# BoloniniD/CSWin-UNet

Hardware: AMD Instinct MI355X
Metric: training images/sec (224x224, cswin_tiny) (higher is better)
Workload: dtype f32; 1 GPU; cswin_tiny_224_lite, synthetic 224x224 9-class, bs=24/GPU, fp32 matmul, fwd + 0.4CE+0.6Dice + bwd + SGD(momentum) step, drop_path 0.2; global_batch=24, img_size=224, parallelism=dp1, hip_graph=True

## Files before the change

### cswin_unet_amd/_lib.py

```python
import ctypes
import os
from ctypes import c_char_p, c_double, c_float, c_int, c_long, c_size_t, c_void_p

import torch

_HERE = os.path.dirname(os.path.abspath(__file__))
LIB_PATH = os.path.join(_HERE, "libcswin_hip.so")

P, I, F, SZ, L, D = c_void_p, c_int, c_float, c_size_t, c_long, c_double

ABI_VERSION = 4

SIGNATURES = {
    "cswin_last_error": (c_char_p, []),
    "cswin_abi_version": (I, []),
    "cswin_device_ok": (I, []),
    "cswin_attn_fwd": (I, [P, P, P, P, P, P, I, I, I, I, P, P, I, F, F, ctypes.c_ulonglong, P, I, P]),
    "cswin_attn_bwd_workspace": (SZ, [I, I, I, I, P, P, I]),
    "cswin_attn_bwd": (I, [P, P, P, P, P, P, P, P, P, P, SZ, I, I, I, I, P, P, I, F, P, F, ctypes.c_ulonglong, P, I, P]),
    "cswin_img2windows": (I, [P, P, I, I, I, I, I, I, P]),
    "cswin_windows2img": (I, [P, P, I, I, I, I, I, I, P]),
    "cswin_layernorm_fwd": (I, [P, P, P, P, P, P, I, I, F, I, P]),
    "cswin_layernorm_bwd_workspace": (SZ, [I, I]),
    "cswin_layernorm_bwd": (I, [P, P, P, P, P, P, P, P, P, P, SZ, I, I, P, P, P]),
    "cswin_linear_fwd": (I, [P, P, I, P, P, P, P, P, P, I, I, I, I, I, I, P]),
    "cswin_linear_bwd_data": (I, [P, P, P, P, I, P, P, I, P, I, I, I, I, I, P]),
    "cswin_linear_bwd_weight_workspace": (SZ, [I, I, I]),
    "cswin_linear_bwd_weight": (I, [P, P, P, I, P, I, P, P, P, SZ, I, I, I, P, I, P]),
    "cswin_linear_bwd_weight_batch": (I, [P, I, P, P, I, P]),
    "cswin_linear_bwd_tail": (I, [P, P, P, I, I, I, P, I, P, P, I, P]),
    "cswin_rows_sum_multi": (I, [P, I, P]),
    "cswin_conv_tok_fwd": (I, [P, P, P, P, I, I, I, I, I, I, I, I, I, P]),
    "cswin_conv_tok_bwd_data": (I, [P, P, P, I, I, I, I, I, I, I, I, I, P]),
    "cswin_conv_tok_bwd_weight_workspace": (SZ, [I, I, I, I, I, I, I, I]),
    "cswin_conv_tok_bwd_weight": (I, [P, P, P, P, P, SZ, I, I, I, I, I, I, I, I, I, P, I, P]),
    "cswin_conv_weight_permute": (I, [P, P, P, I, I, I, I, P]),
    "cswin_conv_weight_unpermute": (I, [P, P, I, I, I, I, P]),
    "cswin_conv_weight_flipT": (I, [P, P, I, I, I, P]),
    "cswin_conv_weight_images": (I, [P, I, P]),
    "cswin_conv_tok_bwd_weight_cpad": (I, [P, P, P, P, P, SZ, I, I, I, I, I, I, I, I, I, P, I, P]),
    "cswin_nchw_to_tokens": (I, [P, P, I, I, I, I, I, P]),
    "cswin_tokens_to_nchw": (I, [P, P, I, I, I, I, I, P]),
    "cswin_carafe_fwd": (I, [P, P, P, P, P, I, I, I, I, I, P]),
    "cswin_carafe_bwd_workspace": (SZ, [I, I, I, I, I]),
    "cswin_carafe_bwd": (I, [P, P, P, P, P, P, P, SZ, I, I, I, I, I, P, P]),
# ... 183 lines not shown
```

### cswin_unet_amd/csrc/gemm.hip

```cpp
#include <stdlib.h>

#include <type_traits>
#include "common.h"
#include "gemm_epilogue.h"

int cswin_gemm16(int mode, int epi_mode, const void* A, const void* B, const void* epilogue, int M, int NO, int R, void* stream);
int cswin_wgrad16_batch(const cswin_wgrad_desc* d, int n, const int* splits, const int* rows_per_split, const cswin_reduce_job* pending,
                        int npending, void* stream, long long* stamps);

namespace {

constexpr int BKMAX = 64;

typedef __bf16 bf16x8 __attribute__((ext_vector_type(8)));
typedef __bf16 bf16x4 __attribute__((ext_vector_type(4)));

#define CSWIN_CHECK_PRECISION(p, who) CSWIN_REQUIRE((p) == 0 || (p) == 1, CSWIN_ERR_UNSUPPORTED, who ": precision %d (0 = fp32, 1 = bf16 operands)", (p))

struct PlainSrc {
    const float* p; long ld; int rows, cols;
    const float* row_scale; int rows_per_sample;
    int bf16;
    static constexpr bool fast_div = false;
    struct Row { const float* base; float s; };
// ... 2 lines not shown
    __device__ Row row(int i) const {
        Row r;
        r.base = (i < rows) ? p + (long)i * ld : nullptr;
        r.s = (row_scale && i < rows) ? row_scale[i / rows_per_sample] : 1.0f;
        return r;
    }
    __device__ const float* ptr(const Row& r, int j) const { return (r.base && j < cols) ? r.base + j : nullptr; }
};

template <class S> __device__ __forceinline__ bool src_is_bf16(const S&) { return false; }
__device__ __forceinline__ bool src_is_bf16(const PlainSrc& s) { return s.bf16 != 0; }
template <class S> __device__ __forceinline__ u32x2 src_load4_bf16(const S&, const float*) { return u32x2{0u, 0u}; }
__device__ __forceinline__ u32x2 src_load4_bf16(const PlainSrc& s, const float* p) {
    return *reinterpret_cast<const u32x2*>(reinterpret_cast<const __bf16*>(s.p) + (p - s.p));
}

struct ConcatSrc {
    const float* p0; const float* p1; long ld0, ld1; int rows, cols, c0;
    static constexpr bool fast_div = false;
    struct Row { const float* b0; const float* b1; float s; };
    typedef int Col;
    __device__ Col col(int j) const { return j; }
    __device__ Row row(int i) const {
        Row r;
        r.b0 = (i < rows) ? p0 + (long)i * ld0 : nullptr;
        r.b1 = (i < rows) ? p1 + (long)i * ld1 : nullptr;
        r.s = 1.0f;
        return r;
    }
    __device__ const float* ptr(const Row& r, int j) const {
// ... 132 lines not shown
        return r;
    }
    __device__ Col col(int j) const { return j; }
    __device__ const float* ptr(const Row& r, int j) const { return (r.base && j < cols) ? r.base + j : nullptr; }
};

template <int BM, int BN, int BK, int KW, bool A_RC, bool B_RC>
constexpr int gemm_lds_floats() {
    constexpr int NW = (BM >= 64 ? 2 : 1) * (BN >= 64 ? 2 : 1);
    constexpr int LDR = BK + 4;
    constexpr int A_ELEMS = A_RC ? BM * LDR : BK * (BM + 4);
    constexpr int B_ELEMS = B_RC ? BN * LDR : BK * (BN + 4);
    return (A_ELEMS + B_ELEMS) > NW * EP_WAVE_FLOATS ? (A_ELEMS + B_ELEMS) : NW * EP_WAVE_FLOATS;
}

template <int BM, int BN, int BK, int KW, bool A_RC, bool B_RC, int VEC, int EPI, bool SCALE_A, int PREC, class ASrc, class BSrc>
__device__ __forceinline__ void gemm_body(float* lds, const ASrc& A, const BSrc& B, const Epilogue& epi, int M, int N, int R,
                                          int r_per_split, int tiles_m, int tiles_n, int bid, int nblk, int stamp_row) {
    constexpr int WGM = BM >= 64 ? 2 : 1, WGN = BN >= 64 ? 2 : 1, NW = WGM * WGN;
    constexpr int WM = BM / WGM, WN = BN / WGN;
    constexpr int FM = WM / 32, FN = WN / 32;
    constexpr int LDR = BK + 4;
    constexpr int LDA = A_RC ? LDR : BM + 4;
    constexpr int LDB = B_RC ? LDR : BN + 4;
    constexpr int A_ELEMS = A_RC ? BM * LDR : BK * (BM + 4);
    constexpr int B_ELEMS = B_RC ? BN * LDR : BK * (BN + 4);
    constexpr int LDS_FLOATS = gemm_lds_floats<BM, BN, BK, KW, A_RC, B_RC>();
    static_assert(LDS_FLOATS >= A_ELEMS + B_ELEMS && LDS_FLOATS >= NW * EP_WAVE_FLOATS, "gemm_lds_floats out of step with the tile geometry");
    float* As = lds;
    float* Bs = lds + A_ELEMS;
    constexpr int LD16 = BK + 8;
    unsigned short* As16 = reinterpret_cast<unsigned short*>(lds);
    unsigned short* Bs16 = As16 + BM * LD16;
    static_assert(PREC == 0 || ((BM + BN) * LD16 * 2 <= LDS_FLOATS * 4 && (BK / KW) % 16 == 0), "bf16 tile does not fit");

    constexpr int NTH = 64 * NW * KW;
    const int tid = threadIdx.x, lane = tid & 63, wave = (tid >> 6) % NW, kg = tid / (64 * NW);
    const int li = lane & 31, lh = lane >> 5;
    const int xq = nblk >> 3, xr = nblk & 7, xcd = bid & 7;
    const int lb = (xcd < xr ? xcd * (xq + 1) : xr * (xq + 1) + (xcd - xr) * xq) + (bid >> 3);
    const int tiles = tiles_m * tiles_n;
    const int split = lb / tiles;
    const int tile = lb - split * tiles;
    const int m0 = (tile / tiles_n) * BM, n0 = (tile % tiles_n) * BN;
    const int r_begin = split * r_per_split;
    const int r_end = min(R, r_begin + r_per_split);
    const int wm0 = (wave / WGN) * WM, wn0 = (wave % WGN) * WN;

    constexpr int QA = BM * BK / (4 * NTH), QB = BN * BK / (4 * NTH);
    static_assert(QA >= 1 && QB >= 1 && (BK / KW) % 8 == 0, "tile too small for this many wave groups");
    constexpr int A_CPR = A_RC ? BK / 4 : BM / 4;
    constexpr int B_CPR = B_RC ? BK / 4 : BN / 4;
    constexpr int A_RPP = NTH / A_CPR, B_RPP = NTH / B_CPR;
    const int a_c = tid % A_CPR, a_r = tid / A_CPR;
    const int b_c = tid % B_CPR, b_r = tid / B_CPR;

    typename ASrc::Row arow[QA];
    typename BSrc::Row brow[QB];
    if (A_RC) {
#pragma unroll
        for (int q = 0; q < QA; ++q) arow[q] = A.row(m0 + a_r + q * A_RPP);
    }
    if (B_RC) {
#pragma unroll
        for (int q = 0; q < QB; ++q) brow[q] = B.row(n0 + b_r + q * B_RPP);
    }

    const typename ASrc::Col acol = A.col(m0 + 4 * a_c);
    const typename BSrc::Col bcol = B.col(n0 + 4 * b_c);

    f32x4 pa[QA], pb[QB];
    u32x2 pa16[QA], pb16[QB];
    float pas[QA];
    auto fetch = [&](int r0, auto a16, auto b16) {
#pragma unroll
        for (int q = 0; q < QA; ++q) {
            typename ASrc::Row rr;
            int j;
            if (A_RC) {
                rr = arow[q];
                j = r0 + 4 * a_c;
            } else {
                const int r = r0 + a_r + q * A_RPP;
                rr = A.row(r < r_end ? r : 0x7fffffff);
                j = m0 + 4 * a_c;
            }
            if (SCALE_A) pas[q] = rr.s;
            if (VEC == 4) {
                const float* p = A_RC ? (j < r_end ? A.ptr(rr, A.col(j)) : nullptr) : A.ptr(rr, acol);
                if constexpr (decltype(a16)::value) {
                    pa16[q] = u32x2{0u, 0u};
                    if (p) pa16[q] = src_load4_bf16(A, p);
                } else {
                    pa[q] = f32x4{0.f, 0.f, 0.f, 0.f};
                    if (p) pa[q] = *reinterpret_cast<const f32x4*>(p);
                }
            } else {
#pragma unroll
                for (int e = 0; e < 4; ++e) {
                    const float* p = (!A_RC || j + e < r_end) ? A.ptr(rr, A.col(j + e)) : nullptr;
                    pa[q][e] = p ? *p : 0.f;
                }
            }
        }
#pragma unroll
        for (int q = 0; q < QB; ++q) {
            typename BSrc::Row rr;
            int j;
            if (B_RC) {
                rr = brow[q];
                j = r0 + 4 * b_c;
            } else {
                const int r = r0 + b_r + q * B_RPP;
                rr = B.row(r < r_end ? r : 0x7fffffff);
                j = n0 + 4 * b_c;
            }
            if (VEC == 4) {
                const float* p = B_RC ? (j < r_end ? B.ptr(rr, B.col(j)) : nullptr) : B.ptr(rr, bcol);
                if constexpr (decltype(b16)::value) {
                    pb16[q] = u32x2{0u, 0u};
                    if (p) pb16[q] = src_load4_bf16(B, p);
                } else {
                    pb[q] = f32x4{0.f, 0.f, 0.f, 0.f};
                    if (p) pb[q] = *reinterpret_cast<const f32x4*>(p);
                }
            } else {
#pragma unroll
                for (int e = 0; e < 4; ++e) {
                    const float* p = (!B_RC || j + e < r_end) ? B.ptr(rr, B.col(j + e)) : nullptr;
// ... 220 lines not shown
                                                    int r_per_split, int tiles_m, int tiles_n) {
    __shared__ __attribute__((aligned(16))) float lds[gemm_lds_floats<BM, BN, BK, KW, A_RC, B_RC>()];
    gemm_body<BM, BN, BK, KW, A_RC, B_RC, VEC, EPI, SCALE_A, PREC, ASrc, BSrc>(lds, A, B, epi, M, N, R, r_per_split, tiles_m, tiles_n,
                                                                              (int)blockIdx.x, (int)gridDim.x, (int)blockIdx.x);
}

constexpr int WGRAD_BATCH = 4;
template <class ASrc, class BSrc>
struct GemmBatch {
    ASrc A[WGRAD_BATCH];
    BSrc B[WGRAD_BATCH];
    Epilogue e[WGRAD_BATCH];
    int M[WGRAD_BATCH], N[WGRAD_BATCH], R[WGRAD_BATCH], rps[WGRAD_BATCH], tm[WGRAD_BATCH], tn[WGRAD_BATCH];
    int first[WGRAD_BATCH + 1];
    int n;
};
typedef GemmBatch<PlainSrc, PlainSrc> WgradBatch;

template <int PREC>
__global__ __launch_bounds__(512) void gemm_wgrad_batch_kernel(WgradBatch b) {
    int p = 0;
    while (p + 1 < b.n && (int)blockIdx.x >= b.first[p + 1]) ++p;
    __shared__ __attribute__((aligned(16))) float lds[gemm_lds_floats<64, 64, 64, 2, false, false>()];
    gemm_body<64, 64, 64, 2, false, false, 4, EPI_PLAIN, true, PREC, PlainSrc, PlainSrc>(
        lds, b.A[p], b.B[p], b.e[p], b.M[p], b.N[p], b.R[p], b.rps[p], b.tm[p], b.tn[p], (int)blockIdx.x - b.first[p],
        b.first[p + 1] - b.first[p], (int)blockIdx.x);
}

struct BlockTail {
    PlainSrc dA, dB;
    Epilogue de;
    int dM, dN, dR, drps, dtm, dtn, nd;
    WgradBatch w;
    ReduceRiders r;
};
__global__ __launch_bounds__(512) void gemm_block_tail_kernel(BlockTail t) {
    constexpr int L0 = gemm_lds_floats<64, 64, 64, 2, true, false>(), L1 = gemm_lds_floats<64, 64, 64, 2, false, false>();
    __shared__ __attribute__((aligned(16))) float lds[L0 > L1 ? L0 : L1];
    const WgradBatch& b = t.w;
    const int nw = b.first[b.n];
    if ((int)blockIdx.x >= nw + t.nd) {
        if (threadIdx.x >= 256) return;
        static_assert(sizeof(lds) >= sizeof(float) * RS_G * (RS_COLS + 1), "reduction scratch");
        rows_sum_dispatch(t.r.j, t.r.first_block, t.r.njobs, (int)blockIdx.x - nw - t.nd, reinterpret_cast<float(*)[RS_COLS + 1]>(lds));
        return;
    }
    if ((int)blockIdx.x >= nw) {
        gemm_body<64, 64, 64, 2, true, false, 4, EPI_PLAIN, false, 0, PlainSrc, PlainSrc>(
            lds, t.dA, t.dB, t.de, t.dM, t.dN, t.dR, t.drps, t.dtm, t.dtn, (int)blockIdx.x - nw, t.nd, (int)blockIdx.x);
        return;
    }
    const int bid = (int)blockIdx.x;
    int p = 0;
    while (p + 1 < b.n && bid >= b.first[p + 1]) ++p;
    gemm_body<64, 64, 64, 2, false, false, 4, EPI_PLAIN, true, 0, PlainSrc, PlainSrc>(
        lds, b.A[p], b.B[p], b.e[p], b.M[p], b.N[p], b.R[p], b.rps[p], b.tm[p], b.tn[p], bid - b.first[p],
        b.first[p + 1] - b.first[p], (int)blockIdx.x);
}

template <int KW, int PREC, bool FAST>
__global__ __launch_bounds__(256 * KW) void gemm_conv_s2_dgrad_batch_kernel(GemmBatch<ConvTS2SrcT<FAST>, TapRowsSrcT<FAST>> b) {
    int p = 0;
    while (p + 1 < b.n && (int)blockIdx.x >= b.first[p + 1]) ++p;
    __shared__ __attribute__((aligned(16))) float lds[gemm_lds_floats<64, 64, (KW == 1 ? 32 : 64), KW, true, false>()];
    gemm_body<64, 64, (KW == 1 ? 32 : 64), KW, true, false, 4, EPI_PLAIN, false, PREC, ConvTS2SrcT<FAST>, TapRowsSrcT<FAST>>(
        lds, b.A[p], b.B[p], b.e[p], b.M[p], b.N[p], b.R[p], b.rps[p], b.tm[p], b.tn[p], (int)blockIdx.x - b.first[p],
        b.first[p + 1] - b.first[p], (int)blockIdx.x);
}

template <int BM, int BN, int BK, int KW, bool A_RC, bool B_RC, int VEC, int EPI, bool SCALE_A, int PREC, class ASrc, class BSrc>
void launch_cfg(const ASrc& A, const BSrc& B, const Epilogue& epi, int M, int N, int R, int splits, int r_per_split,
                hipStream_t st) {
// ... 135 lines not shown
        PlainSrc B = {x, K, M, K, nullptr, 1};
        bool vec = (N % 4 == 0) && (K % 4 == 0) && aligned16(dy) && aligned16(x);
        if (row_scale) launch_gemm_vec<false, false, EPI_PLAIN, true>(vec, A, B, e, N, K, M, splits, rps, precision, st);
        else launch_gemm_vec<false, false, EPI_PLAIN, false>(vec, A, B, e, N, K, M, splits, rps, precision, st);
    }
    CSWIN_LAUNCH_CHECK();
    reduce_now_or_defer(slabs.job(dw, dbias, splits), deferred, st);
    CSWIN_LAUNCH_CHECK();
    return CSWIN_OK;
}

bool wgrad_aligned(const cswin_wgrad_desc& p) {
    return p.N % 4 == 0 && p.K % 4 == 0 && aligned16(p.dy) && aligned16(p.x) && aligned16(p.workspace);
}

struct TailExtras { const char* who; const float* dy; const float* w; float* dx; int M, N, K; const cswin_reduce_job* jobs; int njobs; };

int wgrad_batch_impl(const cswin_wgrad_desc* d, int n, cswin_reduce_job* deferred, const TailExtras& x, void* stream) {
    CSWIN_REQUIRE(x.njobs >= 0 && x.njobs <= CSWIN_TAIL_RIDER_JOBS && (x.njobs == 0 || x.jobs), CSWIN_ERR_SHAPE,
                  "%s: 0..%d pending reductions", x.who, CSWIN_TAIL_RIDER_JOBS);
    CSWIN_REQUIRE(d && deferred && n >= 1 && n <= WGRAD_BATCH, CSWIN_ERR_SHAPE, "linear_bwd_weight_batch: 1..%d problems and their deferred slots", WGRAD_BATCH);
    bool fast = true, any_bf16 = false;
    const int precision = d[0].precision;
    CSWIN_CHECK_PRECISION(precision, "linear_bwd_weight_batch");
    for (int i = 0; i < n; ++i) {
        CSWIN_REQUIRE(d[i].precision == precision, CSWIN_ERR_UNSUPPORTED, "linear_bwd_weight_batch: problems of one launch share one precision");
        CSWIN_REQUIRE(d[i].io_bf16 == 0 || (precision == 1 && (d[i].io_bf16 & ~3) == 0), CSWIN_ERR_UNSUPPORTED, "linear_bwd_weight_batch: bf16 storage needs precision 1");
        CSWIN_REQUIRE(d[i].dy && d[i].x && d[i].dw && d[i].M > 0 && d[i].N > 0 && d[i].K > 0, CSWIN_ERR_SHAPE, "linear_bwd_weight_batch: bad problem %d", i);
        CSWIN_REQUIRE(!d[i].row_scale || d[i].rows_per_sample > 0, CSWIN_ERR_SHAPE, "linear_bwd_weight_batch: rows_per_sample must be > 0");
        size_t need = WgradSlabs::bytes(d[i].M, d[i].N, d[i].K);
        CSWIN_REQUIRE(d[i].workspace && d[i].ws_bytes >= need, CSWIN_ERR_WORKSPACE, "linear_bwd_weight_batch: workspace %zu < %zu", d[i].ws_bytes, need);
        fast = fast && wgrad_aligned(d[i]);
        any_bf16 = any_bf16 || d[i].io_bf16;
    }
    const bool has_dgrad = x.dy != nullptr, extra = has_dgrad || x.njobs > 0;
    const PlainSrc gA = {x.dy, x.N, x.M, x.N, nullptr, 1, 0}, gB = {x.w, x.K, x.N, x.K, nullptr, 1, 0};
    const bool g_vec = x.N % 4 == 0 && x.K % 4 == 0 && aligned16(x.dy) && aligned16(x.w);
    const bool merge_on = cswin_tuning().gemm_tail_merge != 0;
    const bool ride = extra && merge_on && fast && precision == 0 && (!has_dgrad || (g_vec && aligned16(x.dx)));
    const bool w16_path = fast && precision == 1 && (cswin_tuning().wgrad16_on || any_bf16);
    const bool jobs_ride16 = merge_on && w16_path && x.njobs > 0;
    if (extra && !ride) {
        if (has_dgrad) {
            launch_gemm_vec<true, false, EPI_PLAIN, false>(g_vec, gA, gB, plain_epilogue(x.dx, x.K), x.M, x.K, x.N, 1, one_split(x.N), precision,
                                                           (hipStream_t)stream);
            CSWIN_LAUNCH_CHECK();
        }
        if (x.njobs > 0 && !jobs_ride16) {
            int rc = rows_sum_multi(x.jobs, x.njobs, stream);
// ... 45 lines not shown
        int batch_target = total_wgs / n;
        if (!batch_even) {
            double work = 0.0;
            for (int j = 0; j < n; ++j) work += (double)d[j].M * cdiv(d[j].N, 64) * cdiv(d[j].K, 64);
            batch_target = (int)(total_wgs * ((double)M * cdiv(N, 64) * cdiv(K, 64) / work) + 0.5);
            if (batch_target > 1024) batch_target = 1024;
            if (batch_target < 1) batch_target = 1;
        }
        choose_split(M, N, K, &splits, &rps, batch_target);
        const WgradSlabs slabs(d[i].workspace, N, K);
        CSWIN_REQUIRE((size_t)splits * slabs.stride * sizeof(float) <= d[i].ws_bytes, CSWIN_ERR_WORKSPACE,
                      "linear_bwd_weight_batch: %d slabs do not fit problem %d's workspace", splits, i);
        push(b, PlainSrc{d[i].dy, N, M, N, d[i].row_scale, d[i].row_scale ? d[i].rows_per_sample : 1},
             PlainSrc{d[i].x, K, M, K, nullptr, 1}, slabs.epilogue(d[i].dbias != nullptr), N, K, M, rps, splits);
        deferred[i] = slabs.job(d[i].dw, d[i].dbias, splits);
    }
    const int blocks = b.first[n];
    if (ride) {
        BlockTail t = {};
        if (has_dgrad) {
            t.dA = gA; t.dB = gB;
            t.de = plain_epilogue(x.dx, x.K);
            t.de.vec_store = epilogue_vec_ok(t.de, x.K);
            t.dM = x.M; t.dN = x.K; t.dR = x.N; t.drps = one_split(x.N);
            t.dtm = cdiv(x.M, 64); t.dtn = cdiv(x.K, 64);
            t.nd = t.dtm * t.dtn;
        }
        t.w = b;
        int rblocks = 0;
        if (x.njobs > 0) {
            rblocks = fill_reduce_table(x.jobs, x.njobs, t.r.j, t.r.first_block);
            CSWIN_REQUIRE(rblocks >= 0, CSWIN_ERR_SHAPE, "linear_bwd_tail: bad pending reduction");
            t.r.njobs = x.njobs;
        }
        static_assert(sizeof(BlockTail) <= 4096, "kernel argument block");
        hipLaunchKernelGGL(gemm_block_tail_kernel, dim3(blocks + t.nd + rblocks), dim3(512), 0, (hipStream_t)stream, t);
    } else if (precision == 1) {
        hipLaunchKernelGGL(gemm_wgrad_batch_kernel<1>, dim3(blocks), dim3(512), 0, (hipStream_t)stream, b);
    } else {
        hipLaunchKernelGGL(gemm_wgrad_batch_kernel<0>, dim3(blocks), dim3(512), 0, (hipStream_t)stream, b);
    }
    CSWIN_LAUNCH_CHECK();
    return CSWIN_OK;
}

bool conv_magics(ConvMagics* m, long nrows, int img, int w, long ncols, int c, int ks, int cmax, int stride) {
    *m = ConvMagics{fdiv_magic(img), fdiv_magic(w), fdiv_magic(c), fdiv_magic(ks), fdiv_magic(stride)};
    return fdiv_exact(nrows + 63, img) && fdiv_exact(img - 1, w) && fdiv_exact(ncols - 1, c) && fdiv_exact((long)ks * ks - 1, ks) &&
           (stride == 0 || fdiv_exact(cmax, stride));
}
template <class F> void with_fast_div(bool fast, F f) {
// ... 22 lines not shown
        ConvSrcT<decltype(fast)::value> Bm = {x, B, H, W, Cin, OH, OW, ks, stride, pad, M, K, mg};
        launch_gemm<false, false, 4, EPI_PLAIN, false>(A, Bm, slabs.epilogue(dbias != nullptr), Cout, K, M, splits, rps, precision, st);
    });
    CSWIN_LAUNCH_CHECK();
    reduce_now_or_defer(slabs.job(dw_perm, dbias, splits, torch_layout ? ks * ks : 0,
                                  torch_layout ? (Cin | (Cin_param != Cin ? Cin_param << 16 : 0)) : 0), deferred, st);
    CSWIN_LAUNCH_CHECK();
    return CSWIN_OK;
}

}

extern "C" {

void cswin_debug_set_stamps(void* p) { g_stamps = (long long*)p; }

int cswin_linear_fwd(const float* x, const float* x2, int k_split, const float* w, const float* bias, float* y,
                     float* y_act, const float* residual, const float* row_scale, int rows_per_sample, int M, int N,
                     int K, int precision, int io_bf16, void* stream) {
    CSWIN_CHECK_PRECISION(precision, "linear_fwd");
    CSWIN_REQUIRE(io_bf16 == 0 || (precision == 1 && (!x2 || !(io_bf16 & 1)) && (io_bf16 & ~7) == 0 && K % 4 == 0 && N % 4 == 0 && !((io_bf16 & 2) && residual)), CSWIN_ERR_UNSUPPORTED,
                  "linear_fwd: bf16 storage (io_bf16 = %d: 1 = x, 2 = y / y_act, 4 = w) needs precision 1, a plain input for bit 1, K and N multiples of 4; a residual output stays fp32", io_bf16);
    CSWIN_REQUIRE(x && w && y && M > 0 && N > 0 && K > 0, CSWIN_ERR_SHAPE, "linear_fwd: bad arguments M=%d N=%d K=%d", M, N, K);
    CSWIN_REQUIRE(!x2 || (k_split > 0 && k_split < K), CSWIN_ERR_SHAPE, "linear_fwd: bad concat split %d of K=%d", k_split, K);
    CSWIN_REQUIRE(!row_scale || rows_per_sample > 0, CSWIN_ERR_SHAPE, "linear_fwd: rows_per_sample must be > 0");
    hipStream_t st = (hipStream_t)stream;
    Epilogue e = plain_epilogue(y, N);
    e.bias = bias;
    e.Cact = y_act; e.ldact = N;
    e.residual = residual; e.ldres = N;
// ... 81 lines not shown
    hipStream_t st = (hipStream_t)stream;
    const cswin_wgrad_desc d1 = {dy, x, row_scale, dw, dbias, workspace, ws_bytes, rows_per_sample, M, N, K, precision, 0};
    if (precision == 1 && !x2 && wgrad_aligned(d1)) {
        cswin_reduce_job job;
        int rc = wgrad_batch_impl(&d1, 1, &job, TailExtras{"linear_bwd_weight_batch"}, stream);
        if (rc) return rc;
        reduce_now_or_defer(job, deferred, st);
        CSWIN_LAUNCH_CHECK();
        return CSWIN_OK;
    }
    return wgrad_tiled(dy, x, x2, k_split, row_scale, rows_per_sample, dw, dbias, workspace, M, N, K, deferred, precision, st);
}

int cswin_linear_bwd_weight_batch(const cswin_wgrad_desc* d, int n, cswin_reduce_job* deferred, const cswin_reduce_job* pending, int npending,
                                  void* stream) {
    return wgrad_batch_impl(d, n, deferred, TailExtras{"linear_bwd_weight_batch", nullptr, nullptr, nullptr, 0, 0, 0, pending, npending}, stream);
}

int cswin_linear_bwd_tail(const float* dy, const float* w, float* dx, int M, int N, int K, const cswin_wgrad_desc* d, int n,
                          cswin_reduce_job* deferred, const cswin_reduce_job* pending, int npending, void* stream) {
    CSWIN_REQUIRE(dy && w && dx && M > 0 && N > 0 && K > 0, CSWIN_ERR_SHAPE, "linear_bwd_tail: bad data-gradient arguments");
    return wgrad_batch_impl(d, n, deferred, TailExtras{"linear_bwd_tail", dy, w, dx, M, N, K, pending, npending}, stream);
}

int cswin_conv_tok_fwd(const float* x, const float* w_perm, const float* bias, float* y, int B, int H, int W, int Cin,
                       int Cout, int ks, int stride, int pad, int precision, void* stream) {
    CSWIN_CHECK_PRECISION(precision, "conv_tok_fwd");
    CSWIN_REQUIRE(x && w_perm && y && B > 0 && H > 0 && W > 0 && Cin > 0 && Cout > 0, CSWIN_ERR_SHAPE, "conv_tok_fwd: bad arguments");
    CSWIN_REQUIRE(Cin % 4 == 0 && aligned16(x) && aligned16(w_perm), CSWIN_ERR_ALIGN, "conv_tok_fwd: Cin %% 4 and 16-B alignment required");
    int OH = (H + 2 * pad - ks) / stride + 1, OW = (W + 2 * pad - ks) / stride + 1;
    int M = B * OH * OW, R = ks * ks * Cin;
    PlainSrc Bm = {w_perm, R, Cout, R, nullptr, 1};
    Epilogue e = plain_epilogue(y, Cout);
    e.bias = bias;
    ConvMagics mg;
    with_fast_div(conv_magics(&mg, M, OH * OW, OW, R, Cin, ks, 0, 0), [&](auto fast) {
        ConvSrcT<decltype(fast)::value> A = {x, B, H, W, Cin, OH, OW, ks, stride, pad, M, R, mg};
// ... 94 lines not shown
```

### cswin_unet_amd/ops.py

```python
import ctypes
import math

import numpy as np
import torch
from torch.autograd import Function
from torch.autograd.function import once_differentiable

from ._lib import AugmentDesc, ConvImageJob, CswinHipError, ReduceJob, WgradDesc, act_bf16, call, dev_f32, lib, precision, ptr, shadow_ptr, stream

__all__ = ["layer_norm", "linear", "linear_pair", "mlp", "stripe_attention", "cswin_block", "conv_tokens", "patch_embed_conv", "carafe_reassemble",
           "carafe_reassemble_nchw", "conv_weight_images", "head_compose", "tokens_to_nchw", "matmul_nn", "ce_dice_loss", "continual_loss", "dropout", "img2windows", "windows2img",
           "seg_metrics", "resize_slices", "argmax_zoom_back", "augment_batch"]


MAX_REDUCE_JOBS = 48
TAIL_RIDER_JOBS = 16


class engine_backward:

    def __init__(self, opt=None):
        self._flat = opt.flat_grad if opt is not None else None
        self._slots = {p.data_ptr(): (o, p.numel()) for p, o in zip(opt.params, opt.offsets)} if opt is not None else {}
        self._queue = []
# ... 176 lines not shown
    K = K1 + (dx2.shape[-1] if dx2 is not None else 0)
    call("cswin_linear_bwd_data", ptr(dy), pw, ptr(dx), ptr(dx2), K1 if dx2 is not None else 0, ptr(gelu_pre), ptr(row_scale),
         _rows_per_sample(dy), ptr(add), dy.numel() // N, N, K, precision(), _stored16(dy, dx, None, gelu_pre) | w16, stream())


def _linear_bwd_weight(dy, x, dw, db, slab=None, *, x2=None, row_scale=None):
    N, K1 = dy.shape[-1], x.shape[-1]
    K = K1 + (x2.shape[-1] if x2 is not None else 0)
    M = dy.numel() // N
    if slab is None:
        return _reduced(lib().cswin_linear_bwd_weight_workspace(M, N, K), dy.device,
                        lambda *s: _linear_bwd_weight(dy, x, dw, db, s, x2=x2, row_scale=row_scale))
    ws, nbytes, job = slab
    call("cswin_linear_bwd_weight", ptr(dy), ptr(x), ptr(x2), K1 if x2 is not None else 0, ptr(row_scale), _rows_per_sample(dy),
         ptr(dw), ptr(db), ws, nbytes, M, N, K, job, precision(), stream())


def _fill_wgrad(d, dy, x, row_scale, dw, dbias, workspace, ws_bytes):
    d.dy, d.x, d.row_scale, d.dw, d.dbias = (t.data_ptr() if t is not None else None for t in (dy, x, row_scale, dw, dbias))
    d.workspace, d.ws_bytes, d.rows_per_sample = workspace, ws_bytes, _rows_per_sample(dy)
    d.N, d.K = dy.shape[-1], x.shape[-1]
    d.M, d.precision, d.io_bf16 = dy.numel() // d.N, precision(), _stored16(dy, x)


def _linear_bwd_weight_batch(wg, jobs, pending=(None, 0)):
    call("cswin_linear_bwd_weight_batch", ctypes.cast(wg, ctypes.c_void_p), len(wg), _job_ptr(jobs), *pending, stream())


class _Linear(Function):
    @staticmethod
# ... 316 lines not shown
        dwp, dbp = G(kwp, *wp.shape), G(kbp, C)
        _fill_wgrad(wg[2], dx1g, att, rs1, dwp, dbp, wsp[3], sizes[3])
        dqkv = torch.empty_like(qkv)
        dlw = [G(k, *t.shape) for k, t in zip(klepe[:nb], lw)]
        dlb = [G(k, *t.shape) for k, t in zip(klepe[nb:], lb)]
        reso, split, idx, heads = ctx.attn[:4]
        naw = h.cswin_attn_bwd_workspace(B, reso, C, nb, _int_array(heads), _int_array(idx), split)
        aws = _ws(naw, dev)
        _attn_bwd(qkv, lw, lb, lse, att0, datt, dqkv, dlw, dlb, *ctx.attn, (ptr(aws), naw, _job_ptr(jobs, 6)))
        dwqkv, dbqkv = G(kwqkv, *wqkv.shape), G(kbqkv, 3 * C)
        _fill_wgrad(wg[3], dqkv, h1, None, dwqkv, dbqkv, wsp[4], sizes[4])
        wjobs = (ReduceJob * 4)()
        dh1 = datt
        pend, npend, riders = _pass.take_pending()
        if precision() == 0:
            call("cswin_linear_bwd_tail", ptr(dqkv), ptr(wqkv), ptr(dh1), M, 3 * C, C, ctypes.cast(wg, ctypes.c_void_p), 4,
                 _job_ptr(wjobs), pend, npend, stream())
        else:
            _linear_bwd_weight_batch(wg, wjobs, (pend, npend))
            _linear_bwd_data(dqkv, sq, dh1)
        for slot, ji in enumerate((0, 1, 3, 4)):
            jobs[ji] = wjobs[slot]
        dx, dg1, dbt1 = torch.empty_like(x), G(kg1, C), G(kb1, C)
        dx16 = torch.empty_like(x, dtype=torch.bfloat16) if s16 else None
        _layernorm_bwd(dh1, x, m1, r1, g1, dx, dg1, dbt1, (wsp[5], sizes[5], _job_ptr(jobs, 5)), dres=dx1, dx16=dx16)
        if s16:
            _twin_put(dx, dx16)
        _pass.reduce(jobs, (ws, aws))
        grads = (dx, None, None, None, None, None, None, None, None, None, None, dg1, dbt1, dwqkv, dbqkv, dwp, dbp, dg2, dbt2, dw1, db1,
                 dw2, db2)
        return grads + tuple(d.view(d.shape[0], 1, 3, 3) for d in dlw) + tuple(dlb)

# ... 575 lines not shown
```

### include/cswin_hip.h

```cpp
#ifndef CSWIN_HIP_H
#define CSWIN_HIP_H

#include <stddef.h>

#ifdef __cplusplus
extern "C" {
#endif

#define CSWIN_ABI_VERSION 4

#define CSWIN_OK 0
#define CSWIN_ERR_SHAPE (-1)
#define CSWIN_ERR_ALIGN (-2)
#define CSWIN_ERR_WORKSPACE (-3)
#define CSWIN_ERR_HIP (-4)
#define CSWIN_ERR_UNSUPPORTED (-5)

typedef struct cswin_reduce_job {
    const float* part;
    float* out;
    float* out2;
    long long n_first, n, stride;
    int rows, reserved;
    int conv_kk, conv_cin;
// ... 37 lines not shown
    const float* dy;
    const float* x;
    const float* row_scale;
    float* dw;
    float* dbias;
    void* workspace;
    size_t ws_bytes;
    int rows_per_sample, M, N, K;
    int precision;
    int io_bf16;
} cswin_wgrad_desc;
int cswin_linear_bwd_weight_batch(const cswin_wgrad_desc* problems, int n, cswin_reduce_job* deferred, const cswin_reduce_job* pending,
                                  int npending, void* stream);
int cswin_linear_bwd_tail(const float* dy, const float* w, float* dx, int M, int N, int K, const cswin_wgrad_desc* problems, int n,
                          cswin_reduce_job* deferred, const cswin_reduce_job* pending, int npending, void* stream);
int cswin_rows_sum_multi(const cswin_reduce_job* jobs, int njobs, void* stream);

int cswin_conv_tok_fwd(const float* x, const float* w_perm, const float* bias, float* y, int B, int H, int W, int Cin,
                       int Cout, int ks, int stride, int pad, int precision, void* stream);
int cswin_conv_tok_bwd_data(const float* dy, const float* w_permT, float* dx, int B, int H, int W, int Cin, int Cout,
                            int ks, int stride, int pad, int precision, void* stream);
size_t cswin_conv_tok_bwd_weight_workspace(int B, int H, int W, int Cin, int Cout, int ks, int stride, int pad);
int cswin_conv_tok_bwd_weight(const float* dy, const float* x, float* dw, float* dbias, void* workspace,
                              size_t ws_bytes, int B, int H, int W, int Cin, int Cout, int ks, int stride, int pad,
                              int torch_layout, cswin_reduce_job* deferred, int precision, void* stream);
int cswin_conv_weight_permute(const float* w, float* w_perm, float* w_permT, int Cout, int Cin, int ks, int Cpad,
                              void* stream);
int cswin_conv_weight_unpermute(const float* dw_perm, float* dw, int Cout, int Cin, int ks, int Cpad, void* stream);
int cswin_conv_weight_flipT(const float* w, float* wf, int Cout, int Cin, int ks, void* stream);
typedef struct cswin_conv_image_job {
// ... 101 lines not shown
```

Measured before the change: 1934 images/sec.

## Skip drop-path-zeroed samples in weight-gradient GEMMs of the block tail

Adds a masked variant of the batched weight-gradient GEMM. It compacts the list of samples whose drop-path scale is nonzero inside each workgroup and remaps the reduction rows so that dropped samples are never loaded or multiplied. The CSWin block backward uses it for the four wgrad problems when residual scales are present, which avoids spending reduction work on gradients that are known to be zero. In exchange, every block now does a ballot/compaction prologue and an extra division per fetched row. The split sizing is also recomputed at runtime, so the grid is still sized for the full row count and some blocks may end up idle.

```diff
diff --git a/cswin_unet_amd/_lib.py b/cswin_unet_amd/_lib.py
--- a/cswin_unet_amd/_lib.py
+++ b/cswin_unet_amd/_lib.py
@@ -29,6 +29,8 @@
     "cswin_linear_bwd_weight": (I, [P, P, P, I, P, I, P, P, P, SZ, I, I, I, P, I, P]),
     "cswin_linear_bwd_weight_batch": (I, [P, I, P, P, I, P]),
     "cswin_linear_bwd_tail": (I, [P, P, P, I, I, I, P, I, P, P, I, P]),
+    "cswin_linear_bwd_weight_batch_masked": (I, [P, I, P, P, I, P, P, P]),
+    "cswin_linear_bwd_tail_masked": (I, [P, P, P, I, I, I, P, I, P, P, I, P, P, P]),
     "cswin_rows_sum_multi": (I, [P, I, P]),
     "cswin_conv_tok_fwd": (I, [P, P, P, P, I, I, I, I, I, I, I, I, I, P]),
     "cswin_conv_tok_bwd_data": (I, [P, P, P, I, I, I, I, I, I, I, I, I, P]),
diff --git a/cswin_unet_amd/csrc/gemm.hip b/cswin_unet_amd/csrc/gemm.hip
--- a/cswin_unet_amd/csrc/gemm.hip
+++ b/cswin_unet_amd/csrc/gemm.hip
@@ -40,6 +40,15 @@
 __device__ __forceinline__ u32x2 src_load4_bf16(const PlainSrc& s, const float* p) {
     return *reinterpret_cast<const u32x2*>(reinterpret_cast<const __bf16*>(s.p) + (p - s.p));
 }
+template <class S> __device__ __forceinline__ typename S::Row src_mapped_row(const S&, int, float) { return typename S::Row{}; }
+__device__ __forceinline__ PlainSrc::Row src_mapped_row(const PlainSrc& s, int row, float f) {
+    PlainSrc::Row r;
+    r.base = row >= 0 ? s.p + (long)row * s.ld : nullptr;
+    r.s = f;
+    return r;
+}
+template <class S> __device__ __forceinline__ const float* src_row_scale(const S&) { return nullptr; }
+__device__ __forceinline__ const float* src_row_scale(const PlainSrc& s) { return s.row_scale; }
 
 struct ConcatSrc {
     const float* p0; const float* p1; long ld0, ld1; int rows, cols, c0;
@@ -202,9 +211,15 @@
     return (A_ELEMS + B_ELEMS) > NW * EP_WAVE_FLOATS ? (A_ELEMS + B_ELEMS) : NW * EP_WAVE_FLOATS;
 }
 
-template <int BM, int BN, int BK, int KW, bool A_RC, bool B_RC, int VEC, int EPI, bool SCALE_A, int PREC, class ASrc, class BSrc>
+struct RowMask { const float* skip; int nsamples, rows_per_sample, splits; unsigned magic; };
+constexpr int MASK_MAX_SAMPLES = 256;
+struct KeptList { int n; int idx[MASK_MAX_SAMPLES]; float scale[MASK_MAX_SAMPLES]; };
+
+template <int BM, int BN, int BK, int KW, bool A_RC, bool B_RC, int VEC, int EPI, bool SCALE_A, int PREC, class ASrc, class BSrc,
+          bool MASKED = false>
 __device__ __forceinline__ void gemm_body(float* lds, const ASrc& A, const BSrc& B, const Epilogue& epi, int M, int N, int R,
-                                          int r_per_split, int tiles_m, int tiles_n, int bid, int nblk, int stamp_row) {
+                                          int r_per_split, int tiles_m, int tiles_n, int bid, int nblk, int stamp_row,
+                                          const RowMask* mk = nullptr, KeptList* kept = nullptr) {
     constexpr int WGM = BM >= 64 ? 2 : 1, WGN = BN >= 64 ? 2 : 1, NW = WGM * WGN;
     constexpr int WM = BM / WGM, WN = BN / WGN;
     constexpr int FM = WM / 32, FN = WN / 32;
@@ -231,6 +246,28 @@
     const int split = lb / tiles;
     const int tile = lb - split * tiles;
     const int m0 = (tile / tiles_n) * BM, n0 = (tile % tiles_n) * BN;
+    if constexpr (MASKED) {
+        static_assert(!A_RC && !B_RC && VEC == 4 && BM == BN && std::is_same<ASrc, PlainSrc>::value && std::is_same<BSrc, PlainSrc>::value,
+                      "the sample mask serves weight gradients of plain matrices (one row mapping for both operands)");
+        if (tid < 64) {
+            int n = 0;
+            for (int s0 = 0; s0 < mk->nsamples; s0 += 64) {
+                const int s = s0 + lane;
+                const bool keep = s < mk->nsamples && mk->skip[s] != 0.0f;
+                const unsigned long long bal = __ballot(keep);
+                if (keep) {
+                    const int at = n + __popcll(bal & ((1ull << lane) - 1ull));
+                    kept->idx[at] = s;
+                    kept->scale[at] = src_row_scale(A) ? src_row_scale(A)[s] : 1.0f;
+                }
+                n += __popcll(bal);
+            }
+            if (tid == 0) kept->n = n;
+        }
+        __syncthreads();
+        R = __builtin_amdgcn_readfirstlane(kept->n) * mk->rows_per_sample;
+        r_per_split = ((R + mk->splits - 1) / mk->splits + 7) / 8 * 8;
+    }
     const int r_begin = split * r_per_split;
     const int r_end = min(R, r_begin + r_per_split);
     const int wm0 = (wave / WGN) * WM, wn0 = (wave % WGN) * WN;
@@ -261,6 +298,21 @@
     u32x2 pa16[QA], pb16[QB];
     float pas[QA];
     auto fetch = [&](int r0, auto a16, auto b16) {
+        int mrow[QA];
+        float msc[QA];
+        if constexpr (MASKED) {
+#pragma unroll
+            for (int q = 0; q < QA; ++q) {
+                const int c = r0 + a_r + q * A_RPP;
+                mrow[q] = -1;
+                msc[q] = 1.0f;
+                if (c < r_end) {
+                    const int j = fdiv1(c, mk->magic);
+                    mrow[q] = kept->idx[j] * mk->rows_per_sample + (c - j * mk->rows_per_sample);
+                    msc[q] = kept->scale[j];
+                }
+            }
+        }
 #pragma unroll
         for (int q = 0; q < QA; ++q) {
             typename ASrc::Row rr;
@@ -270,7 +322,8 @@
                 j = r0 + 4 * a_c;
             } else {
                 const int r = r0 + a_r + q * A_RPP;
-                rr = A.row(r < r_end ? r : 0x7fffffff);
+                if constexpr (MASKED) rr = src_mapped_row(A, mrow[q], msc[q]);
+                else rr = A.row(r < r_end ? r : 0x7fffffff);
                 j = m0 + 4 * a_c;
             }
             if (SCALE_A) pas[q] = rr.s;
@@ -300,7 +353,8 @@
                 j = r0 + 4 * b_c;
             } else {
                 const int r = r0 + b_r + q * B_RPP;
-                rr = B.row(r < r_end ? r : 0x7fffffff);
+                if constexpr (MASKED) rr = src_mapped_row(B, mrow[q], 1.0f);
+                else rr = B.row(r < r_end ? r : 0x7fffffff);
                 j = n0 + 4 * b_c;
             }
             if (VEC == 4) {
@@ -551,8 +605,21 @@
     int M[WGRAD_BATCH], N[WGRAD_BATCH], R[WGRAD_BATCH], rps[WGRAD_BATCH], tm[WGRAD_BATCH], tn[WGRAD_BATCH];
     int first[WGRAD_BATCH + 1];
     int n;
+    RowMask mask[WGRAD_BATCH];
 };
 typedef GemmBatch<PlainSrc, PlainSrc> WgradBatch;
+
+__device__ __forceinline__ void wgrad_masked_batch_body(float* lds, KeptList* kept, const WgradBatch& b, int p, int bid) {
+    if (b.mask[p].skip) {
+        gemm_body<64, 64, 64, 2, false, false, 4, EPI_PLAIN, true, 0, PlainSrc, PlainSrc, true>(
+            lds, b.A[p], b.B[p], b.e[p], b.M[p], b.N[p], b.R[p], b.rps[p], b.tm[p], b.tn[p], bid - b.first[p],
+            b.first[p + 1] - b.first[p], bid, &b.mask[p], kept);
+        return;
+    }
+    gemm_body<64, 64, 64, 2, false, false, 4, EPI_PLAIN, true, 0, PlainSrc, PlainSrc>(
+        lds, b.A[p], b.B[p], b.e[p], b.M[p], b.N[p], b.R[p], b.rps[p], b.tm[p], b.tn[p], bid - b.first[p],
+        b.first[p + 1] - b.first[p], bid);
+}
 
 template <int PREC>
 __global__ __launch_bounds__(512) void gemm_wgrad_batch_kernel(WgradBatch b) {
@@ -563,6 +630,13 @@
         lds, b.A[p], b.B[p], b.e[p], b.M[p], b.N[p], b.R[p], b.rps[p], b.tm[p], b.tn[p], (int)blockIdx.x - b.first[p],
         b.first[p + 1] - b.first[p], (int)blockIdx.x);
 }
+__global__ __launch_bounds__(512) void gemm_wgrad_batch_masked_kernel(WgradBatch b) {
+    int p = 0;
+    while (p + 1 < b.n && (int)blockIdx.x >= b.first[p + 1]) ++p;
+    __shared__ __attribute__((aligned(16))) float lds[gemm_lds_floats<64, 64, 64, 2, false, false>()];
+    __shared__ KeptList kept;
+    wgrad_masked_batch_body(lds, &kept, b, p, (int)blockIdx.x);
+}
 
 struct BlockTail {
     PlainSrc dA, dB;
@@ -571,9 +645,10 @@
     WgradBatch w;
     ReduceRiders r;
 };
-__global__ __launch_bounds__(512) void gemm_block_tail_kernel(BlockTail t) {
-    constexpr int L0 = gemm_lds_floats<64, 64, 64, 2, true, false>(), L1 = gemm_lds_floats<64, 64, 64, 2, false, false>();
-    __shared__ __attribute__((aligned(16))) float lds[L0 > L1 ? L0 : L1];
+constexpr int BLOCK_TAIL_LDS = gemm_lds_floats<64, 64, 64, 2, true, false>() > gemm_lds_floats<64, 64, 64, 2, false, false>()
+                                   ? gemm_lds_floats<64, 64, 64, 2, true, false>() : gemm_lds_floats<64, 64, 64, 2, false, false>();
+template <bool MASKED>
+__device__ __forceinline__ void block_tail_body(float (&lds)[BLOCK_TAIL_LDS], KeptList* kept, const BlockTail& t) {
     const WgradBatch& b = t.w;
     const int nw = b.first[b.n];
     if ((int)blockIdx.x >= nw + t.nd) {
@@ -590,9 +665,22 @@
     const int bid = (int)blockIdx.x;
     int p = 0;
     while (p + 1 < b.n && bid >= b.first[p + 1]) ++p;
-    gemm_body<64, 64, 64, 2, false, false, 4, EPI_PLAIN, true, 0, PlainSrc, PlainSrc>(
-        lds, b.A[p], b.B[p], b.e[p], b.M[p], b.N[p], b.R[p], b.rps[p], b.tm[p], b.tn[p], bid - b.first[p],
-        b.first[p + 1] - b.first[p], (int)blockIdx.x);
+    if constexpr (MASKED) {
+        wgrad_masked_batch_body(lds, kept, b, p, bid);
+    } else {
+        gemm_body<64, 64, 64, 2, false, false, 4, EPI_PLAIN, true, 0, PlainSrc, PlainSrc>(
+            lds, b.A[p], b.B[p], b.e[p], b.M[p], b.N[p], b.R[p], b.rps[p], b.tm[p], b.tn[p], bid - b.first[p],
+            b.first[p + 1] - b.first[p], (int)blockIdx.x);
+    }
+}
+__global__ __launch_bounds__(512) void gemm_block_tail_kernel(BlockTail t) {
+    __shared__ __attribute__((aligned(16))) float lds[BLOCK_TAIL_LDS];
+    block_tail_body<false>(lds, nullptr, t);
+}
+__global__ __launch_bounds__(512) void gemm_block_tail_masked_kernel(BlockTail t) {
+    __shared__ __attribute__((aligned(16))) float lds[BLOCK_TAIL_LDS];
+    __shared__ KeptList kept;
+    block_tail_body<true>(lds, &kept, t);
 }
 
 template <int KW, int PREC, bool FAST>
@@ -758,13 +846,16 @@
     return p.N % 4 == 0 && p.K % 4 == 0 && aligned16(p.dy) && aligned16(p.x) && aligned16(p.workspace);
 }
 
-struct TailExtras { const char* who; const float* dy; const float* w; float* dx; int M, N, K; const cswin_reduce_job* jobs; int njobs; };
+struct TailExtras {
+    const char* who; const float* dy; const float* w; float* dx; int M, N, K; const cswin_reduce_job* jobs; int njobs;
+    const float* const* skip; const int* nsamples;
+};
 
 int wgrad_batch_impl(const cswin_wgrad_desc* d, int n, cswin_reduce_job* deferred, const TailExtras& x, void* stream) {
     CSWIN_REQUIRE(x.njobs >= 0 && x.njobs <= CSWIN_TAIL_RIDER_JOBS && (x.njobs == 0 || x.jobs), CSWIN_ERR_SHAPE,
                   "%s: 0..%d pending reductions", x.who, CSWIN_TAIL_RIDER_JOBS);
     CSWIN_REQUIRE(d && deferred && n >= 1 && n <= WGRAD_BATCH, CSWIN_ERR_SHAPE, "linear_bwd_weight_batch: 1..%d problems and their deferred slots", WGRAD_BATCH);
-    bool fast = true, any_bf16 = false;
+    bool fast = true, any_bf16 = false, any_mask = false;
     const int precision = d[0].precision;
     CSWIN_CHECK_PRECISION(precision, "linear_bwd_weight_batch");
     for (int i = 0; i < n; ++i) {
@@ -776,7 +867,18 @@
         CSWIN_REQUIRE(d[i].workspace && d[i].ws_bytes >= need, CSWIN_ERR_WORKSPACE, "linear_bwd_weight_batch: workspace %zu < %zu", d[i].ws_bytes, need);
         fast = fast && wgrad_aligned(d[i]);
         any_bf16 = any_bf16 || d[i].io_bf16;
-    }
+        if (x.skip && x.skip[i]) {
+            any_mask = true;
+            CSWIN_REQUIRE(precision == 0, CSWIN_ERR_UNSUPPORTED, "%s: a sample mask needs precision 0", x.who);
+            CSWIN_REQUIRE(x.nsamples && x.nsamples[i] >= 1 && x.nsamples[i] <= MASK_MAX_SAMPLES, CSWIN_ERR_SHAPE,
+                          "%s: problem %d's mask must have 1..%d samples", x.who, i, MASK_MAX_SAMPLES);
+            CSWIN_REQUIRE(d[i].rows_per_sample > 0 && (long)x.nsamples[i] * d[i].rows_per_sample == d[i].M, CSWIN_ERR_SHAPE,
+                          "%s: problem %d's mask: nsamples * rows_per_sample != M", x.who, i);
+            CSWIN_REQUIRE(fdiv_exact(d[i].M, d[i].rows_per_sample), CSWIN_ERR_UNSUPPORTED,
+                          "%s: problem %d's mask: M * rows_per_sample must stay below 2^32", x.who, i);
+        }
+    }
+    CSWIN_REQUIRE(!any_mask || fast, CSWIN_ERR_ALIGN, "%s: a sample mask needs N, K multiples of 4 and 16-B aligned operands", x.who);
     const bool has_dgrad = x.dy != nullptr, extra = has_dgrad || x.njobs > 0;
     const PlainSrc gA = {x.dy, x.N, x.M, x.N, nullptr, 1, 0}, gB = {x.w, x.K, x.N, x.K, nullptr, 1, 0};
     const bool g_vec = x.N % 4 == 0 && x.K % 4 == 0 && aligned16(x.dy) && aligned16(x.w);
@@ -852,6 +954,7 @@
         push(b, PlainSrc{d[i].dy, N, M, N, d[i].row_scale, d[i].row_scale ? d[i].rows_per_sample : 1},
              PlainSrc{d[i].x, K, M, K, nullptr, 1}, slabs.epilogue(d[i].dbias != nullptr), N, K, M, rps, splits);
         deferred[i] = slabs.job(d[i].dw, d[i].dbias, splits);
+        if (x.skip && x.skip[i]) b.mask[i] = RowMask{x.skip[i], x.nsamples[i], d[i].rows_per_sample, splits, fdiv_magic(d[i].rows_per_sample)};
     }
     const int blocks = b.first[n];
     if (ride) {
@@ -872,7 +975,10 @@
             t.r.njobs = x.njobs;
         }
         static_assert(sizeof(BlockTail) <= 4096, "kernel argument block");
-        hipLaunchKernelGGL(gemm_block_tail_kernel, dim3(blocks + t.nd + rblocks), dim3(512), 0, (hipStream_t)stream, t);
+        if (any_mask) hipLaunchKernelGGL(gemm_block_tail_masked_kernel, dim3(blocks + t.nd + rblocks), dim3(512), 0, (hipStream_t)stream, t);
+        else hipLaunchKernelGGL(gemm_block_tail_kernel, dim3(blocks + t.nd + rblocks), dim3(512), 0, (hipStream_t)stream, t);
+    } else if (any_mask) {
+        hipLaunchKernelGGL(gemm_wgrad_batch_masked_kernel, dim3(blocks), dim3(512), 0, (hipStream_t)stream, b);
     } else if (precision == 1) {
         hipLaunchKernelGGL(gemm_wgrad_batch_kernel<1>, dim3(blocks), dim3(512), 0, (hipStream_t)stream, b);
     } else {
@@ -925,6 +1031,12 @@
 extern "C" {
 
 void cswin_debug_set_stamps(void* p) { g_stamps = (long long*)p; }
+
+int cswin_linear_bwd_weight_batch_masked(const cswin_wgrad_desc* d, int n, cswin_reduce_job* deferred, const cswin_reduce_job* pending,
+                                         int npending, const float* const* skip, const int* nsamples, void* stream);
+int cswin_linear_bwd_tail_masked(const float* dy, const float* w, float* dx, int M, int N, int K, const cswin_wgrad_desc* d, int n,
+                                 cswin_reduce_job* deferred, const cswin_reduce_job* pending, int npending, const float* const* skip,
+                                 const int* nsamples, void* stream);
 
 int cswin_linear_fwd(const float* x, const float* x2, int k_split, const float* w, const float* bias, float* y,
                      float* y_act, const float* residual, const float* row_scale, int rows_per_sample, int M, int N,
@@ -1036,13 +1148,25 @@
 
 int cswin_linear_bwd_weight_batch(const cswin_wgrad_desc* d, int n, cswin_reduce_job* deferred, const cswin_reduce_job* pending, int npending,
                                   void* stream) {
-    return wgrad_batch_impl(d, n, deferred, TailExtras{"linear_bwd_weight_batch", nullptr, nullptr, nullptr, 0, 0, 0, pending, npending}, stream);
+    return cswin_linear_bwd_weight_batch_masked(d, n, deferred, pending, npending, nullptr, nullptr, stream);
+}
+
+int cswin_linear_bwd_weight_batch_masked(const cswin_wgrad_desc* d, int n, cswin_reduce_job* deferred, const cswin_reduce_job* pending,
+                                         int npending, const float* const* skip, const int* nsamples, void* stream) {
+    return wgrad_batch_impl(d, n, deferred,
+                            TailExtras{"linear_bwd_weight_batch", nullptr, nullptr, nullptr, 0, 0, 0, pending, npending, skip, nsamples}, stream);
 }
 
 int cswin_linear_bwd_tail(const float* dy, const float* w, float* dx, int M, int N, int K, const cswin_wgrad_desc* d, int n,
                           cswin_reduce_job* deferred, const cswin_reduce_job* pending, int npending, void* stream) {
+    return cswin_linear_bwd_tail_masked(dy, w, dx, M, N, K, d, n, deferred, pending, npending, nullptr, nullptr, stream);
+}
+
+int cswin_linear_bwd_tail_masked(const float* dy, const float* w, float* dx, int M, int N, int K, const cswin_wgrad_desc* d, int n,
+                                 cswin_reduce_job* deferred, const cswin_reduce_job* pending, int npending, const float* const* skip,
+                                 const int* nsamples, void* stream) {
     CSWIN_REQUIRE(dy && w && dx && M > 0 && N > 0 && K > 0, CSWIN_ERR_SHAPE, "linear_bwd_tail: bad data-gradient arguments");
-    return wgrad_batch_impl(d, n, deferred, TailExtras{"linear_bwd_tail", dy, w, dx, M, N, K, pending, npending}, stream);
+    return wgrad_batch_impl(d, n, deferred, TailExtras{"linear_bwd_tail", dy, w, dx, M, N, K, pending, npending, skip, nsamples}, stream);
 }
 
 int cswin_conv_tok_fwd(const float* x, const float* w_perm, const float* bias, float* y, int B, int H, int W, int Cin,
diff --git a/cswin_unet_amd/ops.py b/cswin_unet_amd/ops.py
--- a/cswin_unet_amd/ops.py
+++ b/cswin_unet_amd/ops.py
@@ -214,6 +214,9 @@
     ws, nbytes, job = slab
     call("cswin_linear_bwd_weight", ptr(dy), ptr(x), ptr(x2), K1 if x2 is not None else 0, ptr(row_scale), _rows_per_sample(dy),
          ptr(dw), ptr(db), ws, nbytes, M, N, K, job, precision(), stream())
+
+
+MAX_MASK_SAMPLES = 256
 
 
 def _fill_wgrad(d, dy, x, row_scale, dw, dbias, workspace, ws_bytes):
@@ -560,8 +563,13 @@
         dh1 = datt
         pend, npend, riders = _pass.take_pending()
         if precision() == 0:
-            call("cswin_linear_bwd_tail", ptr(dqkv), ptr(wqkv), ptr(dh1), M, 3 * C, C, ctypes.cast(wg, ctypes.c_void_p), 4,
-                 _job_ptr(wjobs), pend, npend, stream())
+            tail = (ptr(dqkv), ptr(wqkv), ptr(dh1), M, 3 * C, C, ctypes.cast(wg, ctypes.c_void_p), 4, _job_ptr(wjobs), pend, npend)
+            masks = (rs2, rs2, rs1, rs1) if B <= MAX_MASK_SAMPLES else (None,) * 4
+            if any(m is not None for m in masks):
+                skip = (ctypes.c_void_p * 4)(*[m.data_ptr() if m is not None else None for m in masks])
+                call("cswin_linear_bwd_tail_masked", *tail, skip, _int_array([B] * 4), stream())
+            else:
+                call("cswin_linear_bwd_tail", *tail, stream())
         else:
             _linear_bwd_weight_batch(wg, wjobs, (pend, npend))
             _linear_bwd_data(dqkv, sq, dh1)
diff --git a/include/cswin_hip.h b/include/cswin_hip.h
--- a/include/cswin_hip.h
+++ b/include/cswin_hip.h
@@ -75,6 +75,12 @@
                                   int npending, void* stream);
 int cswin_linear_bwd_tail(const float* dy, const float* w, float* dx, int M, int N, int K, const cswin_wgrad_desc* problems, int n,
                           cswin_reduce_job* deferred, const cswin_reduce_job* pending, int npending, void* stream);
+int cswin_linear_bwd_weight_batch_masked(const cswin_wgrad_desc* problems, int n, cswin_reduce_job* deferred,
+                                         const cswin_reduce_job* pending, int npending, const float* const* skip, const int* nsamples,
+                                         void* stream);
+int cswin_linear_bwd_tail_masked(const float* dy, const float* w, float* dx, int M, int N, int K, const cswin_wgrad_desc* problems, int n,
+                                 cswin_reduce_job* deferred, const cswin_reduce_job* pending, int npending, const float* const* skip,
+                                 const int* nsamples, void* stream);
 int cswin_rows_sum_multi(const cswin_reduce_job* jobs, int njobs, void* stream);
 
 int cswin_conv_tok_fwd(const float* x, const float* w_perm, const float* bias, float* y, int B, int H, int W, int Cin,
```

New measurement: 1954 images/sec (median of 6 runs). 1.01x the previous value.
